# jonassibbesen/rpvg

Measured on AMD Instinct MI355X. Metric: read-pairs quantified/sec, higher is better.
Workload: dtype f64

## Files before the change

### rpvg_amd/csrc/bounded_search.hip

```cpp

#include "common.hpp"
#include "search_plan.hpp"

#include <algorithm>
#include <cstdlib>
#include <map>
#include <memory>
#include <mutex>
#include <numeric>

using namespace rpvg_hip_detail;
using namespace rpvg_search;

namespace {
std::mutex g_search_gate_mutex;
const rpvg_hip_ctx * g_search_gate_owner = nullptr;
}

static bool searchLaunchesEarly() {
    static const bool early = RPVG_EXPERIMENT_ENV("RPVG_HIP_SEARCH_LAUNCH_EARLY") != nullptr;
    return early;
}

constexpr uint64_t kSearchGateRows = 1ull << 17;

static void searchGateEnter(rpvg_hip_ctx * ctx, hipStream_t stream, const uint64_t matrix_rows) {
    static const bool open_gate = RPVG_EXPERIMENT_ENV("RPVG_HIP_NO_SEARCH_GATE") != nullptr;
    ctx->search_gate_held = !open_gate && matrix_rows >= kSearchGateRows;
    if (!ctx->search_gate_held) return;
    hipEvent_t previous = nullptr;
    {
        std::lock_guard<std::mutex> lock(g_search_gate_mutex);
        if (g_search_gate_owner && g_search_gate_owner != ctx && g_search_gate_owner->device == ctx->device) {
            previous = g_search_gate_owner->search_done;
            (void) hipStreamWaitEvent(stream, previous, 0);
        }
    }
    if (previous && !searchLaunchesEarly()) (void) waitEvent(previous);
}

static void searchGateLeave(rpvg_hip_ctx * ctx, hipStream_t stream) {
    if (!ctx->search_gate_held) return;
    ctx->search_gate_held = false;
    std::lock_guard<std::mutex> lock(g_search_gate_mutex);
    (void) hipEventRecord(ctx->search_done, stream);
    g_search_gate_owner = ctx;
}

void searchGateForget(const rpvg_hip_ctx * ctx) {
    std::lock_guard<std::mutex> lock(g_search_gate_mutex);
    if (g_search_gate_owner == ctx) g_search_gate_owner = nullptr;
}

struct rpvg_hip_pair_posteriors {
    std::vector<uint64_t> pair_off;
    void * block = nullptr;
    bool block_pinned = false;
    const uint32_t * first = nullptr, * second = nullptr;
    const double * posterior = nullptr;
    ~rpvg_hip_pair_posteriors() {
        if (block && block_pinned) pinnedFree(block);
        else std::free(block);
    }
};

namespace {

constexpr uint32_t kLdsRows = 2048;
constexpr uint32_t kSmallRowLdsCols = 128;
constexpr uint32_t kRowLdsCols = 512;

__device__ __forceinline__ double waveSum(double v) { return waveSumF64(v); }

__device__ __forceinline__ double addLog(const double log_x, const double log_y) {
    return log_x > log_y ? log_x + log1p(exp(log_y - log_x)) : log_y + log1p(exp(log_x - log_y));
}


template <int kBlock, typename ValueFn>
__device__ __forceinline__ double blockLogSumExp(const uint32_t n, ValueFn value, double * scratch) {
    const double lowest = -1.7976931348623157e308;
    const int lane = threadIdx.x & 63, wave = threadIdx.x >> 6;
    double mx = lowest;
    for (uint32_t k = threadIdx.x; k < n; k += kBlock) mx = fmax(mx, value(k));
#pragma unroll
    for (int d = 32; d >= 1; d >>= 1) mx = fmax(mx, __shfl_xor(mx, d, 64));
    __syncthreads();
    if (lane == 0) scratch[wave] = mx;
    __syncthreads();
#pragma unroll
    for (int w2 = 0; w2 < kBlock / 64; ++w2) mx = fmax(mx, scratch[w2]);
    double sum = 0.0;
    for (uint32_t k = threadIdx.x; k < n; k += kBlock) {
        const double v = value(k);
        if (v > lowest) sum += exp(v - mx);
    }
    sum = waveSum(sum);
    __syncthreads();
    if (lane == 0) scratch[wave] = sum;
    __syncthreads();
    double total = 0.0;
#pragma unroll
    for (int w2 = 0; w2 < kBlock / 64; ++w2) total += scratch[w2];
    return (n == 0 || !(mx > lowest)) ? lowest : mx + log(total);
}

struct SearchArgs {
    const uint32_t * order;
    uint32_t count;
    GroupMatricesView g;
    const uint64_t * col_off;
    const uint32_t * col_count;
    const uint64_t * pair_cap_off;
    double min_log_likelihood_diff;
    uint32_t stage_rows;
    uint32_t row_lds_cols;
    double * log_freq;
    double * marginal;
    double * optimistic_raw;
    double * optimistic;
    uint32_t * col_order;
    uint32_t * out_first;
    uint32_t * out_second;
    double * out_value;
    uint32_t * out_count;
    unsigned long long * log_evals;
};

constexpr int kTileFirst = 4;

template <int kGroup>
__device__ __forceinline__ void tilePairSums(const LogTableEntry * lt, const double * lds_count, const double * lds_base, const uint32_t stride,
                                             const double * __restrict__ cnt, const double * __restrict__ nz,
                                             const double * const (&col_a)[kTileFirst], const double * __restrict__ col_b, const uint32_t staged,
// ... 769 lines not shown
        pair_off[m] = run;
        run += counts[m];
    }
    if (threadIdx.x == 1023) pair_off[num_matrices] = sums[1023];
    if (threadIdx.x == 0 && build_error) *build_error_out = *build_error;
    __syncthreads();
    for (uint32_t i = threadIdx.x; i < tail_words; i += blockDim.x) tail_copy[i] = counts[i];
}

__global__ void compactPairsBlockKernel(const uint32_t num_matrices, const uint64_t * __restrict__ pair_cap_off,
                                        const uint64_t * __restrict__ pair_off, const uint32_t * __restrict__ in_first,
                                        const uint32_t * __restrict__ in_second, const double * __restrict__ in_value,
                                        unsigned char * __restrict__ block) {
    const uint32_t m = blockIdx.x;
    if (m >= num_matrices) return;
    const uint64_t total = pair_off[num_matrices];
    double * out_value = reinterpret_cast<double *>(block);
    uint32_t * out_first = reinterpret_cast<uint32_t *>(block + total * sizeof(double));
    uint32_t * out_second = out_first + total;
    const uint64_t src = pair_cap_off[m], dst = pair_off[m], n = pair_off[m + 1] - pair_off[m];
    for (uint64_t k = threadIdx.x; k < n; k += blockDim.x) {
        out_first[dst + k] = in_first[src + k];
        out_second[dst + k] = in_second[src + k];
        out_value[dst + k] = in_value[src + k];
    }
}


PairSearchKnobs pairSearchKnobs() {
    PairSearchKnobs knobs;
    if (const char * env = std::getenv("RPVG_HIP_PAIR_TILES")) knobs.tiles_wanted = std::atoi(env);
    if (const char * env = std::getenv("RPVG_HIP_TABLE_MIN_WORK")) knobs.table_min_work = std::atof(env);
    if (const char * env = std::getenv("RPVG_HIP_PAIR_CHUNK_ROWS")) knobs.chunk_rows = std::max(256, std::atoi(env));
    return knobs;
}

int searchFailed(const hipError_t e) {
    setError("rpvg_hip_bounded_pair_posteriors: %s", hipGetErrorString(e));
    return (e == hipErrorOutOfMemory) ? RPVG_HIP_ERR_ALLOC : RPVG_HIP_ERR_RUNTIME;
}

void showSearchClasses(const rpvg_hip_groups * groups, const PairSearchPlan & plan) {
    const std::vector<uint32_t> & order = plan.order;
    const uint32_t M = static_cast<uint32_t>(order.size()), num_big = plan.num_big, num_medium = plan.num_medium;
    auto show = [&](const char * name, uint32_t first, uint32_t count) {
        double evals = 0;
        for (uint32_t i = first; i < first + count; ++i) evals += 0.5 * groups->h_num_rows[order[i]] * groups->h_num_cols[order[i]] * groups->h_num_cols[order[i]];
        std::fprintf(stderr, "[search classes] %-6s %6u matrices, %.3g pair-row evaluations if nothing is skipped; largest:", name, count, evals);
        for (uint32_t i = first; i < first + std::min<uint32_t>(count, 6); ++i) std::fprintf(stderr, " %llux%u", static_cast<unsigned long long>(groups->h_num_rows[order[i]]), groups->h_num_cols[order[i]]);
        std::fprintf(stderr, "\n");
    };
    show("table", 0, num_big);
    if (plan.pair_tiles) {
        struct Bucket { uint64_t matrices = 0; double rows = 0, evals = 0, lane_rows = 0, slot_rows = 0; };
        std::map<uint32_t, Bucket> buckets;
        for (uint32_t i = 0; i < num_big; ++i) {
            const double R = static_cast<double>(groups->h_num_rows[order[i]]);
            const uint32_t G = groups->h_num_cols[order[i]];
            uint32_t key = 1;
            while (key < G) key <<= 1;
            Bucket & b = buckets[key];
            const uint32_t tiles = tileCount(G);
            b.matrices += 1;
            b.rows += R;
            b.evals += R * (0.5 * G * (G + 1));
            std::vector<std::pair<uint32_t, uint32_t> > ranges;
            planTileRanges(tiles, &ranges);
            for (auto & range : ranges) b.lane_rows += R / (kTileBlock / range.second) * kTileBlock;
            b.slot_rows += R * tiles * 16;
        }
        for (auto & kv : buckets) {
            const Bucket & b = kv.second;
            std::fprintf(stderr, "[search classes]   columns <= %4u: %6llu matrices, %9.0f rows, %.3g evaluations, pairs / tile slots %.2f, tile slots / lane slots %.2f\n",
                         kv.first, static_cast<unsigned long long>(b.matrices), b.rows, b.evals, b.evals / b.slot_rows, b.slot_rows / (16.0 * b.lane_rows));
        }
    }
    show("medium", num_big, num_medium);
    show("small", num_big + num_medium, M - num_big - num_medium);
}

unsigned long long * searchLogEvals(const PairSearchWork & w) { return reinterpret_cast<unsigned long long *>(w.d_tail.ptr + w.evals_word); }

hipError_t launchTablePart(rpvg_hip_ctx * ctx, const rpvg_hip_groups * groups, const GroupMatricesView & view, const PairSearchPlan & plan,
                           PairSearchWork & w, const bool runs_behind_search) {
    hipError_t e = hipSuccess;
    auto ok = [&](hipError_t r) { if (e == hipSuccess) e = r; return e == hipSuccess; };
    hipStream_t st = ctx->stream;
    const SearchParts parts = {w.d_part_pair.ptr, w.d_part_marg.ptr, w.d_part_opt.ptr, w.d_big_pair_part_off.ptr, w.d_big_col_part_off.ptr, plan.chunk_rows};
    const uint32_t items = static_cast<uint32_t>(plan.item_matrix.size());
    if (plan.pair_tiles) {
        PairTileWork pw;
        pw.item_matrix = w.d_item_matrix.ptr;
        pw.item_chunk = w.d_item_chunk.ptr;
        pw.item_tiles = w.d_item_col.ptr;
        pw.count = items;
        pw.g = view;
        pw.parts = parts;
        pw.log_evals = searchLogEvals(w);
#ifdef RPVG_HIP_EXPERIMENTS
        pw.debug_skip = RPVG_EXPERIMENT_ENV("RPVG_HIP_PAIR_DEBUG") ? static_cast<uint32_t>(std::atoi(RPVG_EXPERIMENT_ENV("RPVG_HIP_PAIR_DEBUG"))) : 0u;
#endif
        static const size_t tile_lds_bytes = []() {
            const char * env = RPVG_EXPERIMENT_ENV("RPVG_HIP_PAIR_LDS_KB");
            return std::max<size_t>(kTileLdsDoubles * sizeof(double), env ? static_cast<size_t>(std::atoi(env)) * 1024 : 0);
        }();
        if (tile_lds_bytes > 64 * 1024) {
            e = hipFuncSetAttribute(reinterpret_cast<const void *>(&pairTile2Kernel), hipFuncAttributeMaxDynamicSharedMemorySize, static_cast<int>(tile_lds_bytes));
            if (e != hipSuccess) return e;
        }
        const int tile_span = ctx->spanBegin(FAM_TILE, st);
        pairTile2Kernel<<<dim3(pw.count), dim3(kTileBlock), tile_lds_bytes, st>>>(pw);
        ctx->spanEnd(tile_span);
#ifdef RPVG_HIP_EXPERIMENTS
        for (int k = RPVG_EXPERIMENT_ENV("RPVG_HIP_PAIR_REPEAT") ? std::atoi(RPVG_EXPERIMENT_ENV("RPVG_HIP_PAIR_REPEAT")) : 0; k > 0; --k) {
            pairTile2Kernel<<<dim3(pw.count), dim3(kTileBlock), tile_lds_bytes, st>>>(pw);
        }
#endif
    } else {
        TableWork tw;
        tw.item_matrix = w.d_item_matrix.ptr;
        tw.item_col = w.d_item_col.ptr;
        tw.item_chunk = w.d_item_chunk.ptr;
        tw.count = items;
        tw.g = view;
        tw.parts = parts;
        tw.log_evals = searchLogEvals(w);
        pairTableKernel<<<dim3(((tw.count + 7) / 8) * 8), dim3(256), 0, st>>>(tw);
    }
    if (runs_behind_search) {
        if (groups->collapse_done) {
            HostScope wait_scope("search: wait for the runs of the matrices' collapse");
            ok(searchLaunchesEarly() ? hipStreamWaitEvent(st, groups->collapse_done, 0) : waitEvent(groups->collapse_done));
        }
        ok(groups->held_back_runs(st, &parts));
        groups->held_back_runs = nullptr;
    }

    ResolveArgs ra;
    ra.big_matrix = w.d_order.ptr;
    ra.count = plan.num_big;
    ra.g = view;
    ra.col_off = w.d_col_off.ptr;
    ra.col_count = w.d_col_count.ptr;
    ra.pair_cap_off = w.d_pair_cap_off.ptr;
    ra.parts = parts;
    ra.min_log_likelihood_diff = w.min_log_likelihood_diff;
    ra.log_freq = w.d_lf.ptr;
    ra.marginal = w.d_marg.ptr;
    ra.col_order = w.d_col_order.ptr;
    ra.seq_value = w.d_seq.ptr;
    ra.out_first = w.d_out_first.ptr;
    ra.out_second = w.d_out_second.ptr;
    ra.out_value = w.d_out_value.ptr;
    ra.out_count = w.d_tail.ptr;
    resolveTableKernel<<<dim3(plan.num_big), dim3(256), 0, st>>>(ra);
    return e;
}

void launchSequentialParts(rpvg_hip_ctx * ctx, const GroupMatricesView & view, const PairSearchPlan & plan, PairSearchWork & w) {
    static const int search_streams = []() {
        const char * env = RPVG_EXPERIMENT_ENV("RPVG_HIP_SEARCH_STREAMS");
        return env ? std::max(1, std::min(3, std::atoi(env))) : 3;
    }();
    hipStream_t s_medium = search_streams == 1 ? ctx->stream : ctx->aux[0];
    hipStream_t s_small = search_streams == 1 ? ctx->stream : (search_streams == 2 ? ctx->aux[0] : ctx->aux[1]);
    SearchArgs args;
    args.g = view;
    args.col_off = w.d_col_off.ptr;
    args.col_count = w.d_col_count.ptr;
    args.pair_cap_off = w.d_pair_cap_off.ptr;
    args.min_log_likelihood_diff = w.min_log_likelihood_diff;
    args.log_freq = w.d_lf.ptr;
    args.marginal = w.d_marg.ptr;
    args.optimistic_raw = w.d_opt_raw.ptr;
    args.optimistic = w.d_opt.ptr;
    args.col_order = w.d_col_order.ptr;
    args.out_first = w.d_out_first.ptr;
    args.out_second = w.d_out_second.ptr;
    args.out_value = w.d_out_value.ptr;
    args.out_count = w.d_tail.ptr;
    args.log_evals = searchLogEvals(w);
    auto search_lds_bytes = [](uint32_t stage_rows, uint32_t row_cols) { return static_cast<size_t>((kTileFirst + 1) * stage_rows + kTileFirst * row_cols) * sizeof(double); };
    {
        static std::once_flag once;
        std::call_once(once, [&]() {
            (void) hipFuncSetAttribute(reinterpret_cast<const void *>(&boundedSearchKernel<1024, 64>), hipFuncAttributeMaxDynamicSharedMemorySize,
                                       static_cast<int>(search_lds_bytes(kLdsRows, kRowLdsCols)));
        });
    }
    const uint32_t num_small = w.M - plan.num_big - plan.num_medium;
    if (plan.num_medium > 0) {
        args.order = w.d_order.ptr + plan.num_big;
        args.count = plan.num_medium;
        args.stage_rows = kLdsRows;
        args.row_lds_cols = kRowLdsCols;
        boundedSearchKernel<1024, 64><<<dim3(plan.num_medium), dim3(1024), search_lds_bytes(kLdsRows, kRowLdsCols), s_medium>>>(args);
    }
    if (num_small > 0) {
        args.order = w.d_order.ptr + plan.num_big + plan.num_medium;
        args.count = num_small;
        args.stage_rows = kSmallRows;
        args.row_lds_cols = kSmallRowLdsCols;
        boundedSearchKernel<256, 16><<<dim3(num_small), dim3(256), search_lds_bytes(kSmallRows, kSmallRowLdsCols), s_small>>>(args);
    }
}

}

namespace rpvg_hip_detail {

int queuePairSearch(rpvg_hip_ctx * ctx, const rpvg_hip_groups * groups, const uint32_t * column_counts, const double min_rel_likelihood,
                    PairSearchWork & w) {
    std::unique_ptr<HostScope> scope(new HostScope("bounded search: host order + work items"));
    const uint32_t M = groups->num_matrices;
    w.M = M;
    w.min_log_likelihood_diff = std::log(min_rel_likelihood);
    if (!column_counts && M > 0 && !groups->d_column_counts) {
        setError("rpvg_hip_bounded_pair_posteriors: column_counts is NULL");
        return RPVG_HIP_ERR_INVALID;
    }
    const uint64_t num_columns = std::accumulate(groups->h_num_cols.begin(), groups->h_num_cols.begin() + M, uint64_t(0));
    for (uint64_t c = 0; column_counts && c < num_columns; ++c) {
        if (column_counts[c] == 0) {
            setError("rpvg_hip_bounded_pair_posteriors: column %llu has a zero count", static_cast<unsigned long long>(c));
            return RPVG_HIP_ERR_INVALID;
        }
    }
    w.plan = planPairSearch(groups->h_num_rows.data(), groups->h_num_cols.data(), M, min_rel_likelihood, pairSearchKnobs());
    const PairSearchPlan & plan = w.plan;
    if (RPVG_EXPERIMENT_ENV("RPVG_HIP_SEARCH_CLASSES")) showSearchClasses(groups, plan);

    scope.reset(new HostScope("bounded search: uploads + launches"));
    hipError_t e = hipSetDevice(ctx->device);
    hipStream_t st = ctx->stream;
    auto ok = [&](hipError_t r) { if (e == hipSuccess) e = r; return e == hipSuccess; };

    UploadPack & pack = w.pack;
    const uint64_t columns = plan.col_off[M], pair_cap = plan.pair_cap_off[M];
    pack.add(w.d_order, plan.order.data(), M);
    pack.add(w.d_col_off, plan.col_off.data(), M + 1);
    pack.add(w.d_pair_cap_off, plan.pair_cap_off.data(), M + 1);
    if (column_counts) pack.add(w.d_col_count, column_counts, columns);
    if (plan.num_big > 0) {
        pack.add(w.d_item_matrix, plan.item_matrix.data(), plan.item_matrix.size());
        pack.add(w.d_item_col, plan.item_col.data(), plan.item_col.size());
        pack.add(w.d_item_chunk, plan.item_chunk.data(), plan.item_chunk.size());
        pack.add(w.d_big_col_part_off, plan.big_col_part_off.data(), M);
        pack.add(w.d_big_pair_part_off, plan.big_pair_part_off.data(), M);
    }
    w.evals_word = (M + 1) & ~1u;
    w.tail_words = w.evals_word + 4;
    pack.addZero(w.d_tail, w.tail_words);
    if (w.extra_u64_count) pack.add(w.d_extra_u64, w.extra_u64, w.extra_u64_count);
    if (w.extra_zero_bytes) pack.addZero(w.d_extra_zero, w.extra_zero_bytes);
    int span = ctx->spanBegin(FAM_H2D);
    ok(pack.commit(st));
    if (!column_counts) w.d_col_count.borrow(const_cast<uint32_t *>(groups->d_column_counts), columns);
    ctx->spanEnd(span);
    ctx->stats.h2d_bytes += static_cast<double>(M * 20 + columns * 4);
    ok(w.d_lf.alloc(columns));
    ok(w.d_marg.alloc(columns));
    ok(w.d_opt_raw.alloc(columns));
    ok(w.d_opt.alloc(columns));
    ok(w.d_col_order.alloc(columns));
    ok(w.d_out_first.alloc(pair_cap));
    ok(w.d_out_second.alloc(pair_cap));
    ok(w.d_out_value.alloc(pair_cap));
    if (e != hipSuccess) return searchFailed(e);
    if (plan.num_big > 0) {
        ok(w.d_part_marg.alloc(plan.col_part_total));
        ok(w.d_part_opt.alloc(plan.col_part_total));
        ok(w.d_part_pair.alloc(plan.pair_part_total));
        ok(w.d_seq.alloc(pair_cap));
    }
    if (e != hipSuccess) return searchFailed(e);

    const bool side_kernels = M > plan.num_big;
    const bool runs_behind_search = static_cast<bool>(groups->held_back_runs) && plan.pair_tiles && plan.num_big == M;
    if (!runs_behind_search) {
        ok(groups->waitCollapse(st));
        if (groups->collapse_done && !searchLaunchesEarly()) {
            HostScope wait_scope("search: wait for the collapse of the matrices");
            ok(waitEvent(groups->collapse_done));
        }
    }
    span = ctx->spanBegin(FAM_LOGLIK);
    searchGateEnter(ctx, st, std::accumulate(groups->h_num_rows.begin(), groups->h_num_rows.end(), uint64_t(0)));
    if (side_kernels) ok(ctx->forkAux());
    const GroupMatricesView view = groups->view();
    if (plan.num_big > 0) ok(launchTablePart(ctx, groups, view, plan, w, runs_behind_search && e == hipSuccess));
    launchSequentialParts(ctx, view, plan, w);
    if (side_kernels) ok(ctx->joinAux());
    ctx->spanEnd(span);
    ctx->stats.loglik_launches += (plan.num_big > 0 ? 2 : 0) + (plan.num_medium > 0) + (M > plan.num_big + plan.num_medium);
    ok(hipGetLastError());
    if (e != hipSuccess) {
        (void) hipStreamSynchronize(st);
        searchFailed(e);
        return RPVG_HIP_ERR_RUNTIME;
    }
    return RPVG_HIP_OK;
}

void leavePairSearch(rpvg_hip_ctx * ctx) { searchGateLeave(ctx, ctx->stream); }

void accountPairSearch(rpvg_hip_ctx * ctx, const rpvg_hip_groups * groups, const PairSearchWork & w, const unsigned long long log_evals,
                       const uint64_t kept_pairs) {
    ctx->stats.loglik_evals += static_cast<double>(log_evals);
    for (uint32_t i = 0; i < w.M; ++i) {
        const double G = groups->h_num_cols[w.plan.order[i]];
        ctx->stats.search_pairs_possible += G * (G + 1) / 2;
        if (i < w.plan.num_big) ctx->stats.search_pairs_table += G * (G + 1) / 2;
    }
    ctx->stats.search_pairs_kept += static_cast<double>(kept_pairs);
}

}

extern "C" int rpvg_hip_bounded_pair_posteriors(rpvg_hip_ctx * ctx, const rpvg_hip_groups * groups,
                                                const uint32_t * column_counts, double min_rel_likelihood,
                                                rpvg_hip_pair_posteriors ** result_out) {
    RPVG_REQUIRE(ctx && groups && result_out, "rpvg_hip_bounded_pair_posteriors: NULL argument");
    *result_out = nullptr;
    RPVG_REQUIRE(min_rel_likelihood > 0, "rpvg_hip_bounded_pair_posteriors: min_rel_likelihood must be positive");
    const uint32_t M = groups->num_matrices;
    rpvg_hip_pair_posteriors * res = new (std::nothrow) rpvg_hip_pair_posteriors();
    if (!res) {
        setError("rpvg_hip_bounded_pair_posteriors: out of host memory");
        return RPVG_HIP_ERR_ALLOC;
    }
    res->pair_off.assign(M + 1, 0);
    if (M == 0) {
        *result_out = res;
        return RPVG_HIP_OK;
    }
    if (!column_counts && !groups->d_column_counts) {
        delete res;
        setError("rpvg_hip_bounded_pair_posteriors: column_counts is NULL");
        return RPVG_HIP_ERR_INVALID;
    }

    std::lock_guard<std::mutex> lock(ctx->mutex);
    PairSearchWork w;
    {
        const int rc = queuePairSearch(ctx, groups, column_counts, min_rel_likelihood, w);
        if (rc != RPVG_HIP_OK) {
            delete res;
            return rc;
        }
    }
    hipError_t e = hipSuccess;
    hipStream_t st = ctx->stream;
    auto ok = [&](hipError_t r) { if (e == hipSuccess) e = r; return e == hipSuccess; };
    std::unique_ptr<HostScope> scope;
    const std::vector<uint64_t> & pair_cap_off = w.plan.pair_cap_off;
    const uint32_t evals_word = w.evals_word, tail_words = w.tail_words;
    auto & d_tail = w.d_tail; auto & d_pair_cap_off = w.d_pair_cap_off; auto & d_out_first = w.d_out_first;
    auto & d_out_second = w.d_out_second; auto & d_out_value = w.d_out_value;
    DeviceBuffer<uint64_t> d_pair_off;

    const char * with_counts_env = std::getenv("RPVG_HIP_PAIRS_WITH_COUNTS");
    const size_t kPairsWithTheCounts = with_counts_env ? static_cast<size_t>(std::atof(with_counts_env)) : (size_t(1) << 20);
    const size_t tail_bytes = tail_words * sizeof(uint32_t), tail_room = (tail_bytes + 255) & ~size_t(255);
    const size_t block_capacity = static_cast<size_t>(pair_cap_off[M]) * 16;
    const size_t first_copy = tail_room + std::min(block_capacity, kPairsWithTheCounts);
    DeviceBuffer<unsigned char> d_result;
    ok(d_pair_off.alloc(M + 1));
    ok(d_result.alloc(tail_room + block_capacity));
    void * host_result = nullptr;
    if (e == hipSuccess && pinnedAlloc(&host_result, first_copy) != hipSuccess) e = hipErrorOutOfMemory;
    if (e == hipSuccess) {
        const bool check_build = !groups->build_checked && groups->build_error_flag.ptr;
        pairOffsetsKernel<<<dim3(1), dim3(1024), 0, st>>>(M, d_tail.ptr, d_pair_off.ptr, check_build ? groups->build_error_flag.ptr : nullptr,
                                                         d_tail.ptr + evals_word + 2, reinterpret_cast<uint32_t *>(d_result.ptr), tail_words);
        compactPairsBlockKernel<<<dim3(M), dim3(64), 0, st>>>(M, d_pair_cap_off.ptr, d_pair_off.ptr, d_out_first.ptr, d_out_second.ptr,
                                                             d_out_value.ptr, d_result.ptr + tail_room);
        ok(hipGetLastError());
        ok(hipMemcpyAsync(host_result, d_result.ptr, first_copy, hipMemcpyDeviceToHost, st));
    }
    searchGateLeave(ctx, st);
    scope.reset(new HostScope("bounded search: wait for the kernels"));
    ok(waitStream(st));
    if (e == hipSuccess) {
        const uint32_t * counts = static_cast<const uint32_t *>(host_result);
        unsigned long long log_evals = 0;
        std::memcpy(&log_evals, counts + evals_word, sizeof(log_evals));
        const uint32_t build_bad = counts[evals_word + 2];
        for (uint32_t m = 0; m < M; ++m) res->pair_off[m + 1] = res->pair_off[m] + counts[m];
        if (build_bad) {
            pinnedFree(host_result);
            delete res;
            setError(build_bad == 2 ? "rpvg_hip_groups_build: a group lists a path twice" : "rpvg_hip_groups_build: a group refers to a path outside its cluster");
            return RPVG_HIP_ERR_INVALID;
        }
        groups->build_checked = true;
        const uint64_t total = res->pair_off[M];
        const unsigned char * pairs = nullptr;
        if (total * 16 <= first_copy - tail_room) {
            res->block = host_result;
            res->block_pinned = true;
            host_result = nullptr;
            pairs = static_cast<const unsigned char *>(res->block) + tail_room;
        } else {
            scope.reset(new HostScope("bounded search: download pairs"));
            if (pinnedAlloc(&res->block, total * 16) == hipSuccess) {
                res->block_pinned = true;
            } else {
                res->block = std::malloc(total * 16);
                if (!res->block) e = hipErrorOutOfMemory;
            }
            if (e == hipSuccess) {
                ok(hipMemcpyAsync(res->block, d_result.ptr + tail_room, total * 16, hipMemcpyDeviceToHost, st));
                ok(waitStream(st));
                pairs = static_cast<const unsigned char *>(res->block);
            }
        }
        if (e == hipSuccess) {
            res->posterior = reinterpret_cast<const double *>(pairs);
            res->first = reinterpret_cast<const uint32_t *>(pairs + total * sizeof(double));
            res->second = res->first + total;
        }
        accountPairSearch(ctx, groups, w, log_evals, total);
    }
    if (host_result) pinnedFree(host_result);
    if (e != hipSuccess) {
        delete res;
        return searchFailed(e);
    }
    *result_out = res;
    return RPVG_HIP_OK;
}

extern "C" int rpvg_hip_pair_posteriors_get(const rpvg_hip_pair_posteriors * result, rpvg_hip_pair_posteriors_view * view_out) {
    RPVG_REQUIRE(result && view_out, "rpvg_hip_pair_posteriors_get: NULL argument");
    view_out->num_matrices = static_cast<uint32_t>(result->pair_off.size() - 1);
    view_out->pair_off = result->pair_off.data();
    view_out->first = result->first;
    view_out->second = result->second;
    view_out->posterior = result->posterior;
    return RPVG_HIP_OK;
}

extern "C" void rpvg_hip_pair_posteriors_free(rpvg_hip_pair_posteriors * result) { delete result; }
```

### rpvg_amd/csrc/common.hpp

```cpp
#ifndef RPVG_HIP_COMMON_HPP
#define RPVG_HIP_COMMON_HPP

#include <hip/hip_runtime.h>

#include <algorithm>
#include <chrono>
#include <cstdarg>
#include <cstdint>
#include <cstdio>
#include <cstdlib>
#include <cstring>
#include <memory>
#include <mutex>
#include <new>
#include <string>
#include <functional>
#include <vector>

#include "../../include/rpvg_hip.h"
#include "search_plan.hpp"
#include "em_plan.hpp"
#include "batch_forms.hpp"

namespace rpvg_hip_detail {
// ... 417 lines not shown
        for (int t = 0; t < kOut; ++t) acc[t] = fma(c, logPositive(xs[t], lt), acc[t]);
    }
}

constexpr int kCollapseKeyFractionBits = 22;
constexpr int kCollapseProjectionBits = kCollapseKeyFractionBits + 2;
constexpr int kCollapseLargestBits = 20;
constexpr int kCollapseLargestFractionBits = 27;
constexpr int kCollapseMatrixShift = kCollapseProjectionBits + kCollapseLargestBits;
constexpr uint32_t kCollapseMaxMatrices = 1u << 20;

__host__ __device__ inline double collapseWeight(const uint32_t column) {
    return static_cast<double>(((column * 0x9E3779B1u) >> 8) & 0xFFFFu) * (1.0 / 32768.0);
}

__host__ __device__ inline uint64_t collapseSortKey(const uint32_t matrix, const double key, const double largest) {
    const double k = key < 0.0 ? 0.0 : (key > 3.999999 ? 3.999999 : key);
    const double l = largest < 0.0 ? 0.0 : (largest > 0.999999 ? 0.999999 : largest);
    return (static_cast<uint64_t>(matrix) << kCollapseMatrixShift) |
           (static_cast<uint64_t>(k * static_cast<double>(1ull << kCollapseKeyFractionBits)) << kCollapseLargestBits) |
           (static_cast<uint64_t>(l * static_cast<double>(1ull << kCollapseLargestFractionBits)) & ((1ull << kCollapseLargestBits) - 1));
}

__device__ __forceinline__ double mulRounded(const double a, const double b) {
#pragma clang fp contract(off)
    return a * b;
}
__device__ __forceinline__ double addRounded(const double a, const double b) {
#pragma clang fp contract(off)
    return a + b;
}

template <int BLOCK>
__device__ __forceinline__ uint32_t blockExclusiveSum(const uint32_t v, uint32_t & total, uint32_t * scratch) {
    const int lane = threadIdx.x & 63, wave = threadIdx.x >> 6;
    uint32_t incl = v;
#pragma unroll
    for (int d = 1; d < 64; d <<= 1) {
        const uint32_t up = __shfl_up(incl, d, 64);
        if (lane >= d) incl += up;
    }
    __syncthreads();
    if (lane == 63) scratch[wave] = incl;
    __syncthreads();
    uint32_t before = 0, all = 0;
#pragma unroll
    for (int w = 0; w < BLOCK / 64; ++w) {
        if (w < wave) before += scratch[w];
        all += scratch[w];
    }
    total = all;
    return before + incl - v;
}

enum KernelFamily { FAM_EM_SPARSE = 0, FAM_EM_DENSE, FAM_LOGLIK, FAM_BUILD, FAM_H2D, FAM_COLLAPSE, FAM_EM_KERNEL, FAM_GIBBS, FAM_TILE, FAM_COUNT };

struct TimedSpan {
    hipEvent_t start, stop;
    int family;
    int sub;
};

struct TimedInterval {
    double start_ms, stop_ms;
    int family;
    uint64_t clock;
};

}

namespace rpvg_hip_detail {
struct SubsetEmHints {
    double subsets_per_matrix = 0, list_per_path = 0, rows_per_row = 0, entries_per_entry = 0;
    bool retry = false;
    unsigned long long retry_subsets = 0, retry_list_length = 0, retry_rows = 0, retry_entries = 0;
};
}

struct rpvg_hip_ctx {
    static constexpr int kAuxStreams = 6;
    rpvg_hip_detail::SubsetEmHints subset_hints;
    rpvg_hip_detail::SubsetEmHints subset_full_hints;
    bool search_gate_held = false;
    int device = 0;
    hipStream_t stream = nullptr;
    hipStream_t aux[kAuxStreams] = {};
    int aux_count = kAuxStreams;
    hipStream_t grid_stream[2] = {nullptr, nullptr};
    hipEvent_t grid_ready = nullptr;
    hipStream_t collapse_stream = nullptr;
    hipStream_t copy_stream = nullptr;
    hipEvent_t copied = nullptr;
    hipEvent_t fork_event = nullptr;
    hipEvent_t search_done = nullptr;
    hipEvent_t join_event[kAuxStreams] = {};
    hipError_t forkAux();
    hipError_t joinAux();
    hipError_t joinAuxOnHost();
    hipDeviceProp_t props;
    std::mutex mutex;
    void * comm = nullptr;
    int comm_world = 1, comm_rank = 0;
    int allReduceSumF64(double * device_buf, uint64_t n);
    std::vector<rpvg_hip_detail::TimedSpan> spans;
    std::vector<hipStream_t> span_streams;
    int span_level = 2;
    int open_spans = 0;
    void accountSpan(const rpvg_hip_detail::TimedSpan & span, const void * clock_base, uint64_t clock_id);
    void foldFinishedSpans();
    std::vector<rpvg_hip_detail::TimedInterval> intervals;
    rpvg_hip_kernel_stats stats;

    int spanBegin(int family, hipStream_t on = nullptr, int sub = -1);
    void spanEnd(int idx);
    int foldSpans();
};

namespace rpvg_hip_detail {
struct PathSourcesPending {
    DeviceBuffer<uint64_t> d_path_source_off;
    DeviceBuffer<uint32_t> d_source_id, d_sizes;
    DeviceBuffer<uint16_t> d_source_id16;
    DeviceBuffer<unsigned long long> d_arena;
    unsigned long long arena_words = 0, num_sources = 0, num_sources_narrow = 0;
    void * h_sizes = nullptr;
    uint32_t K = 0;
    bool copied = false, queued = false;
    ~PathSourcesPending() { if (h_sizes) pinnedFree(h_sizes); }
};
}

struct rpvg_hip_batch {
    uint32_t num_clusters = 0;
    uint64_t num_rows = 0, num_entries = 0, num_paths = 0;
    std::vector<uint64_t> h_cluster_row_off, h_cluster_path_off, h_cluster_ent_off;
    rpvg_hip_detail::DeviceBuffer<uint64_t> cluster_row_off;
    rpvg_hip_detail::DeviceBuffer<uint64_t> cluster_path_off;
    rpvg_hip_detail::DeviceBuffer<double> row_count;
    rpvg_hip_detail::DeviceBuffer<double> row_noise;
    rpvg_hip_detail::DeviceBuffer<uint64_t> row_ent_off;
    rpvg_hip_detail::DeviceBuffer<uint32_t> ent_path;
    rpvg_hip_detail::DeviceBuffer<double> ent_prob;
    std::vector<double> h_cluster_total;
    bool has_source_columns = false;
    rpvg_hip_detail::DeviceBuffer<uint32_t> path_group_id;
    rpvg_hip_detail::DeviceBuffer<uint64_t> cluster_src_off;
    rpvg_hip_detail::DeviceBuffer<uint32_t> src_col_count;
    rpvg_hip_detail::DeviceBuffer<uint32_t> src_col_end;
    rpvg_hip_detail::DeviceBuffer<uint32_t> src_col_path;
    std::vector<uint64_t> h_cluster_src_off;
    std::vector<uint32_t> h_src_num_cols, h_src_col_paths, h_src_max_col_paths;
    struct UploadInProgress {
        rpvg_batch_forms::BatchForms forms;
        rpvg_hip_detail::DeviceBuffer<uint32_t> d_row_count_u32, d_row_grp_off32, d_grp_idx_off32;
        rpvg_hip_detail::DeviceBuffer<uint64_t> d_row_grp_off, d_grp_idx_off;
        rpvg_hip_detail::DeviceBuffer<double> d_grp_prob;
        rpvg_hip_detail::DeviceBuffer<uint8_t> d_row_grp_count8, d_grp_idx_count8;
        rpvg_hip_detail::DeviceBuffer<uint16_t> d_path_idx16, d_row_noise16;
        rpvg_hip_detail::DeviceBuffer<double> d_row_noise_table;
        rpvg_hip_detail::DeviceBuffer<uint8_t> d_row_count8;
        rpvg_hip_detail::DeviceBuffer<uint32_t> d_escape_row, d_escape_count;
        rpvg_hip_detail::PathSourcesPending path_sources;
        rpvg_hip_detail::DeviceBuffer<unsigned long long> d_first_bad_row;
        rpvg_hip_detail::DeviceBuffer<double> d_cluster_total;
        rpvg_hip_detail::DeviceBuffer<uint64_t> d_cluster_ent_off;
        rpvg_hip_detail::DeviceBuffer<unsigned char> scan_scratch_rows, scan_scratch_groups;
// ... 240 lines not shown
    EmProblemsView problems;
    double * abundances;
    double * noise_count;
    uint32_t * iterations;
    const EmFusedDense * fused = nullptr;
    uint32_t num_fused = 0;
};

uint64_t emGridMinWork();
uint64_t gibbsGridMinWork();
bool emGridDenseRoute(uint32_t columns, uint32_t rows, uint32_t entries);
int runEmGridProblems(rpvg_hip_ctx * ctx, hipStream_t st, const EmGridProblem * problems, uint32_t count, const EmGridStorage & storage,
                      uint32_t max_em_its, double max_rel_em_conv);

struct GibbsGridProblem {
    uint32_t problem, columns;
    uint32_t rows, entries;
    uint32_t num_samples, pad;
    uint64_t col_begin;
    uint64_t sample_off, abund_sample_off;
    uint64_t seed;
};
struct GibbsGridStorage {
    EmProblemsView problems;
    const double * init_abundances;
    const double * init_noise_count;
    double * noise_samples;
    double * abundance_samples;
};
int runGibbsGridProblems(rpvg_hip_ctx * ctx, hipStream_t st, const GibbsGridProblem * problems, uint32_t count, const GibbsGridStorage & storage,
                         uint32_t gibbs_thin_its, double gamma);

struct DenseEmRun {
    const double * matrix = nullptr;
    uint64_t num_rows = 0;
    uint32_t num_cols = 0;
    uint64_t ld = 0;
    const double * counts = nullptr;
    double total_count = 0, zero_mass = 0;
    uint32_t max_em_its = 0;
    double max_rel_em_conv = 0;
    bool sharded = false;
    DeviceBuffer<double> d_a;
    EmGridControl control = {};
};
int emDenseIterate(rpvg_hip_ctx * ctx, const char * who, DenseEmRun & run);

int queueEmSolve(rpvg_hip_ctx * ctx, const rpvg_hip_batch * batch, const EmProblemList & list, uint32_t max_em_its,
                 double max_rel_em_conv, const EmOutputs & out, EmSolveWork & work, double collapse_precision = 0.0);
EmSolveKnobs emSolveKnobs();
int queueEmFill(rpvg_hip_ctx * ctx, const rpvg_hip_batch * batch, const EmProblemList & list, const EmOutputs & out, EmSolveWork & work,
                const EmSolveKnobs & knobs, const EmFillPlan & plan, bool fused_look, int & build_span);
EmSolveShape emSolveShape(const rpvg_hip_ctx * ctx, const EmProblemList & list, bool collapse_wanted);

struct HostProblemSet {
    EmProblemList list;
    EmSolveWork work;
    DeviceBuffer<uint32_t> d_cluster, d_col_path, d_item_problem;
    DeviceBuffer<uint64_t> d_col_off, d_row_base, d_ent_base, d_seg_first;
    UploadPack uploads;
    uint64_t n_cols_total = 0;
};
int prepareHostProblems(rpvg_hip_ctx * ctx, const rpvg_hip_batch * batch, const rpvg_hip_em_problems * problems,
                        HostProblemSet & ps, const EmOutputs & out, const char * who);
void accountEmSolve(rpvg_hip_ctx * ctx, uint32_t P, const uint64_t * col_off, const uint32_t * kept_rows, const uint32_t * kept_entries,
                    const uint32_t * iterations);

struct PairSearchWork {
    uint32_t M = 0, evals_word = 0, tail_words = 0;
    double min_log_likelihood_diff = 0;
    rpvg_search::PairSearchPlan plan;
    DeviceBuffer<uint32_t> d_order, d_col_count, d_col_order, d_out_first, d_out_second, d_item_matrix, d_item_col, d_item_chunk;
    DeviceBuffer<uint32_t> d_tail;
    DeviceBuffer<uint64_t> d_col_off, d_pair_cap_off, d_big_col_part_off, d_big_pair_part_off;
    DeviceBuffer<double> d_lf, d_marg, d_opt_raw, d_opt, d_out_value, d_part_marg, d_part_opt, d_part_pair, d_seq;
    UploadPack pack;
    const uint64_t * extra_u64 = nullptr;
    size_t extra_u64_count = 0, extra_zero_bytes = 0;
    DeviceBuffer<uint64_t> d_extra_u64;
    DeviceBuffer<unsigned char> d_extra_zero;
};
int queuePairSearch(rpvg_hip_ctx * ctx, const rpvg_hip_groups * groups, const uint32_t * column_counts, double min_rel_likelihood,
                    PairSearchWork & w);
void leavePairSearch(rpvg_hip_ctx * ctx);
void accountPairSearch(rpvg_hip_ctx * ctx, const rpvg_hip_groups * groups, const PairSearchWork & w, unsigned long long log_evals, uint64_t kept_pairs);

struct CsrCollapseInput {
    uint32_t num_problems_bound = 0;
    const uint32_t * num_problems_dev = nullptr;
    uint64_t rows_capacity = 0;
    EmProblemsView problems;
    uint32_t num_items_bound = 0;
    const uint32_t * num_items_dev = nullptr;
    const uint64_t * seg_first = nullptr;
    const uint32_t * item_problem = nullptr;
    uint32_t segment_rows = 0;
    uint64_t max_rows_bound = 0;
};
struct CsrCollapseWork {
    DeviceBuffer<double> merged_count;
    DeviceBuffer<uint32_t> problem_merged;
    DeviceBuffer<uint32_t> info;
    std::shared_ptr<void> temporaries;
};
hipError_t queueCsrCollapse(rpvg_hip_ctx * ctx, const CsrCollapseInput & in, double precision, CsrCollapseWork & work, hipStream_t stream,
                            hipEvent_t sorted = nullptr);

std::unique_ptr<rpvg_hip_batch> newBatchShell(uint32_t num_clusters, uint64_t num_rows, uint64_t num_entries, uint64_t num_paths, hipError_t & e);
struct GroupedRows {
    uint64_t num_groups = 0;
    const void * row_grp_off = nullptr;
    const void * grp_idx_off = nullptr;
    bool row_off32 = false, grp_off32 = false;
    const double * grp_prob = nullptr;
    const uint32_t * row_count_u32 = nullptr;
};
hipError_t queueGroupedRows(hipStream_t stream, const GroupedRows & rows, rpvg_hip_batch * b, unsigned long long * d_first_bad_row, uint64_t * d_cluster_ent_off);

hipError_t queueClusterTotals(hipStream_t stream, uint32_t num_clusters, const uint64_t * d_cluster_row_off, const uint32_t * d_row_count_u32, double * d_totals);
hipError_t queuePathSourceCopies(rpvg_hip_ctx * ctx, rpvg_hip_batch * b, const rpvg_cluster_batch * hb, PathSourcesPending & pending);
hipError_t queuePathSourceKernels(rpvg_hip_ctx * ctx, rpvg_hip_batch * b, PathSourcesPending & pending, hipStream_t stream);
hipError_t reservePathSources(rpvg_hip_batch * b, uint32_t num_clusters, uint64_t num_paths, uint64_t num_sources, PathSourcesPending & pending);
int finishPathSources(rpvg_hip_batch * b, PathSourcesPending & pending);

hipError_t queueRowCollapse(rpvg_hip_ctx * ctx, rpvg_hip_groups * groups, uint64_t total_rows, double precision, hipStream_t stream, bool hold_back_runs = false);
}

#endif
```

### rpvg_amd/csrc/subset_em.hip

```cpp

#include "common.hpp"
#include "subset_pack.hpp"

#include <cmath>
#include <memory>

using namespace rpvg_hip_detail;

namespace {

constexpr uint32_t kMaxSelected = 1024;

struct MergedList {
    const uint32_t * a;
    const uint32_t * b;
    uint32_t na, nb, i, j;
    __device__ __forceinline__ MergedList(const uint32_t * a_in, uint32_t na_in, const uint32_t * b_in, uint32_t nb_in)
        : a(a_in), b(b_in), na(na_in), nb(nb_in), i(0), j(0) {}
    __device__ __forceinline__ bool done() const { return i >= na && j >= nb; }
    __device__ __forceinline__ uint32_t next() {
        if (j >= nb || (i < na && a[i] <= b[j])) return a[i++];
        return b[j++];
    }
};
// ... 539 lines not shown
        cap_subsets = std::min<unsigned long long>(slots, std::max(cap_subsets, hints.retry_subsets + 64));
        cap_length = std::max(cap_length, hints.retry_list_length + 64);
        cap_rows = std::max(cap_rows, hints.retry_rows + 64);
        cap_entries = std::max(cap_entries, hints.retry_entries + 64);
        hints.retry = false;
    }
    const unsigned long long cap_columns = cap_length;
    const unsigned long long cap_items = cap_rows / emFillSegmentRows() + cap_subsets;

    scope.reset(new HostScope("subset em: search + kernels queued"));
    const size_t header_room = 256;
    int rc = RPVG_HIP_OK;
    if (!second_attempt) {
        search.extra_u64 = slot_off.data();
        search.extra_u64_count = M + 1;
        search.extra_zero_bytes = header_room + emQueuesBytes();
        rc = queuePairSearch(ctx, groups, column_counts, min_rel_likelihood, search);
        if (rc != RPVG_HIP_OK) return rc;
    } else {
        const hipError_t zeroed = zeroAsync(search.d_extra_zero.ptr, search.extra_zero_bytes, st);
        if (zeroed != hipSuccess) {
            setError("rpvg_hip_nested_subset_em: %s", hipGetErrorString(zeroed));
            return RPVG_HIP_ERR_RUNTIME;
        }
    }

    hipError_t e = hipSuccess;
    auto ok = [&](hipError_t r) { if (e == hipSuccess) e = r; return e == hipSuccess; };
    const uint64_t * d_slot_off = search.d_extra_u64.ptr;
    SubsetHeader * header = reinterpret_cast<SubsetHeader *>(search.d_extra_zero.ptr);
    static_assert(sizeof(SubsetHeader) <= 256, "room for the header");
    DeviceBuffer<uint32_t> d_slot_first, d_slot_second, d_slot_length, d_slot_columns;
    DeviceBuffer<double> d_slot_weight;
    DeviceBuffer<unsigned char> d_totals, d_bases, d_packed;
    ok(d_slot_first.alloc(slots));
    ok(d_slot_second.alloc(slots));
    ok(d_slot_length.alloc(slots));
    ok(d_slot_columns.alloc(slots));
    ok(d_slot_weight.alloc(slots));
    ok(d_totals.alloc(sizeof(MatrixTotals) * M));
    ok(d_bases.alloc(sizeof(MatrixTotals) * M));
    DeviceBuffer<uint32_t> d_big_matrices;
    ok(d_big_matrices.alloc(M));
    DeviceBuffer<uint32_t> d_sub_cluster, d_path, d_col_path, d_iters, d_kept_rows, d_kept_entries;
    DeviceBuffer<double> d_sub_weight, d_abund, d_noise, d_total;
    DeviceBuffer<uint64_t> d_path_off, d_col_off, d_row_base, d_ent_base, d_subset_off, d_seg_first;
    DeviceBuffer<uint32_t> d_item_problem;
    ok(d_sub_cluster.alloc(cap_subsets));
    ok(d_sub_weight.alloc(cap_subsets));
    ok(d_path_off.alloc(cap_subsets + 1));
    ok(d_col_off.alloc(cap_subsets + 1));
    ok(d_row_base.alloc(cap_subsets));
    ok(d_ent_base.alloc(cap_subsets));
    ok(d_subset_off.alloc(M + 1));
    ok(d_seg_first.alloc(cap_subsets + 1));
    ok(d_item_problem.alloc(cap_items));
    ok(d_path.alloc(cap_length));
    ok(d_col_path.alloc(cap_columns));
    ok(d_abund.alloc(cap_columns));
    ok(d_noise.alloc(cap_subsets));
    ok(d_total.alloc(cap_subsets));
    ok(d_iters.alloc(cap_subsets));
    ok(d_kept_rows.alloc(cap_subsets));
    ok(d_kept_entries.alloc(cap_subsets));
    const size_t packed_capacity = packedLayout(M, cap_subsets, cap_length, cap_columns).bytes;
    ok(d_packed.alloc(packed_capacity));
    const bool merge_here = batch->path_group_id.ptr != nullptr && max_paths < (1u << kMergePathBits) - 2;
    DeviceBuffer<unsigned long long> d_merge_key;
    DeviceBuffer<uint32_t> d_merge_pos;
    DeviceBuffer<double> d_merge_a0, d_merge_a1;
    if (merge_here) {
        ok(d_merge_key.alloc(2 * cap_length + 2));
        ok(d_merge_pos.alloc(2 * cap_length + 2));
        ok(d_merge_a0.alloc(cap_length));
        ok(d_merge_a1.alloc(cap_length));
    }
    void * pinned_header = nullptr;
    if (e == hipSuccess && pinnedAlloc(&pinned_header, sizeof(SubsetHeader)) != hipSuccess) e = hipErrorOutOfMemory;
    hipEvent_t header_here = nullptr;
    if (e == hipSuccess) ok(hipEventCreateWithFlags(&header_here, hipEventDisableTiming));
    if (e != hipSuccess) {
        setError("rpvg_hip_nested_subset_em: %s", hipGetErrorString(e));
        (void) hipStreamSynchronize(st);
        leavePairSearch(ctx);
        if (pinned_header) pinnedFree(pinned_header);
        if (header_here) (void) hipEventDestroy(header_here);
        return (e == hipErrorOutOfMemory) ? RPVG_HIP_ERR_ALLOC : RPVG_HIP_ERR_RUNTIME;
    }
    MatrixTotals * totals = reinterpret_cast<MatrixTotals *>(d_totals.ptr);
    MatrixTotals * bases = reinterpret_cast<MatrixTotals *>(d_bases.ptr);

    std::unique_ptr<HostScope> part_scope(new HostScope("subset em: select + offsets + expand queued"));
    int span = ctx->spanBegin(FAM_BUILD);
    SelectArgs sa;
    sa.num_matrices = M;
    sa.pair_count = search.d_tail.ptr;
    sa.pair_cap_off = search.d_pair_cap_off.ptr;
    sa.pair_first = search.d_out_first.ptr;
    sa.pair_second = search.d_out_second.ptr;
    sa.pair_value = search.d_out_value.ptr;
    sa.group_off = groups->d_group_off;
    sa.group_path_off = groups->d_group_path_off;
    sa.group_path = groups->d_group_path;
    sa.cluster = groups->d_cluster;
    sa.mat_rows = groups->mat_rows.ptr;
    sa.cluster_row_off = batch->cluster_row_off.ptr;
    sa.row_ent_off = batch->row_ent_off.ptr;
    sa.slot_off = d_slot_off;
    sa.min_hap_prob = min_hap_prob;
    sa.segment_rows = emFillSegmentRows();
    sa.slot_first = d_slot_first.ptr;
    sa.slot_second = d_slot_second.ptr;
    sa.slot_weight = d_slot_weight.ptr;
    sa.slot_length = d_slot_length.ptr;
    sa.slot_columns = d_slot_columns.ptr;
    sa.totals = totals;
    sa.header = header;
    sa.big_matrices = d_big_matrices.ptr;
    subsetSelectSmallKernel<<<dim3(M), dim3(64), 0, st>>>(sa);
    subsetSelectWideKernel<<<dim3(std::min<uint32_t>(M, 128)), dim3(256), 0, st>>>(sa);
    const bool check_build = !groups->build_checked && groups->build_error_flag.ptr;
    OffsetsArgs oa;
    oa.pair_count = search.d_tail.ptr;
    oa.log_evals = reinterpret_cast<const unsigned long long *>(search.d_tail.ptr + search.evals_word);
    oa.build_error = check_build ? groups->build_error_flag.ptr : nullptr;
    oa.num_matrices = M;
    oa.totals = totals;
    oa.bases = bases;
    oa.header = header;
    oa.cap_subsets = cap_subsets;
    oa.cap_length = cap_length;
    oa.cap_columns = cap_columns;
    oa.cap_rows = cap_rows;
    oa.cap_entries = cap_entries;
    oa.cap_items = cap_items;
    oa.seg_first = d_seg_first.ptr;
    oa.path_off = d_path_off.ptr;
    oa.col_off = d_col_off.ptr;
    subsetOffsetsKernel<<<dim3(1), dim3(1024), 0, st>>>(oa);
    SubsetHeader * h_header = static_cast<SubsetHeader *>(pinned_header);
    ok(hipMemcpyAsync(h_header, header, sizeof(SubsetHeader), hipMemcpyDeviceToHost, st));
    ok(hipEventRecord(header_here, st));
    ExpandArgs ea;
    ea.num_matrices = M;
    ea.header = header;
    ea.totals = totals;
    ea.bases = bases;
    ea.slot_off = d_slot_off;
    ea.slot_first = d_slot_first.ptr;
    ea.slot_second = d_slot_second.ptr;
    ea.slot_weight = d_slot_weight.ptr;
    ea.slot_length = d_slot_length.ptr;
    ea.slot_columns = d_slot_columns.ptr;
    ea.group_off = groups->d_group_off;
    ea.group_path_off = groups->d_group_path_off;
    ea.group_path = groups->d_group_path;
    ea.cluster = groups->d_cluster;
    ea.cluster_row_off = batch->cluster_row_off.ptr;
    ea.row_ent_off = batch->row_ent_off.ptr;
    ea.sub_cluster = d_sub_cluster.ptr;
    ea.sub_weight = d_sub_weight.ptr;
    ea.path_off = d_path_off.ptr;
    ea.path = d_path.ptr;
    ea.col_off = d_col_off.ptr;
    ea.col_path = d_col_path.ptr;
    ea.row_base = d_row_base.ptr;
    ea.ent_base = d_ent_base.ptr;
    ea.seg_first = d_seg_first.ptr;
    ea.item_problem = d_item_problem.ptr;
    ea.segment_rows = emFillSegmentRows();
    ea.subset_off = d_subset_off.ptr;
    subsetExpandKernel<<<dim3(M), dim3(256), 0, st>>>(ea);
    ok(hipGetLastError());
    ctx->spanEnd(span);
    ctx->stats.build_launches += 4;
    leavePairSearch(ctx);

    part_scope.reset();
    EmProblemList list;
    list.P_bound = static_cast<uint32_t>(std::min<unsigned long long>(cap_subsets, 0xfffffffeull));
    list.d_num_problems = &header->num_problems;
    list.d_cluster = d_sub_cluster.ptr;
    list.d_col_off = d_col_off.ptr;
    list.d_col_path = d_col_path.ptr;
    list.d_row_base = d_row_base.ptr;
    list.d_ent_base = d_ent_base.ptr;
    list.rows_capacity = cap_rows;
    list.entries_capacity = cap_entries;
    list.d_seg_first = d_seg_first.ptr;
    list.d_item_problem = d_item_problem.ptr;
    list.items_bound = static_cast<uint32_t>(std::min<unsigned long long>(cap_items, 0xfffffffeull));
    list.d_num_items = &header->num_items;
    list.max_cols = max_paths + 1;
    list.max_cluster_paths = max_paths;
    list.max_cluster_work = max_cluster_work;
    list.wide_capacity = 0;
    EmOutputs out{d_abund.ptr, d_noise.ptr, d_iters.ptr, d_kept_rows.ptr, d_kept_entries.ptr, d_total.ptr};
    EmSolveWork work;
    work.zeroed_queues = search.d_extra_zero.ptr + header_room;
    if (e == hipSuccess) {
        rc = queueEmSolve(ctx, batch, list, max_em_its, max_rel_em_conv, out, work, collapse_precision);
        if (rc != RPVG_HIP_OK) {
            (void) hipStreamSynchronize(st);
            (void) hipEventDestroy(header_here);
            pinnedFree(pinned_header);
            return rc;
        }
    }
    part_scope.reset(new HostScope("subset em: merge + pack queued"));
    static_assert(sizeof(SubsetHeader) <= 192, "the merge's flag word sits behind the header");
    uint32_t * d_merge_bad = reinterpret_cast<uint32_t *>(search.d_extra_zero.ptr + 192);
    if (merge_here && e == hipSuccess) {
        MergeArgs ma;
        ma.header = header;
        ma.num_matrices = M;
        ma.subset_off = d_subset_off.ptr;
        ma.weight = d_sub_weight.ptr;
        ma.path_off = d_path_off.ptr;
        ma.path = d_path.ptr;
        ma.col_off = d_col_off.ptr;
        ma.col_path = d_col_path.ptr;
        ma.abundances = d_abund.ptr;
        ma.noise = d_noise.ptr;
        ma.total = d_total.ptr;
        ma.cluster = groups->d_cluster;
        ma.cluster_path_off = batch->cluster_path_off.ptr;
        ma.path_group_id = batch->path_group_id.ptr;
        ma.sort_key = d_merge_key.ptr;
        ma.sort_pos = d_merge_pos.ptr;
        ma.rec_a0 = d_merge_a0.ptr;
        ma.rec_a1 = d_merge_a1.ptr;
        ma.merge_bad = d_merge_bad;
        ma.packed = d_packed.ptr;
        const int merge_span = ctx->spanBegin(FAM_BUILD);
        subsetMergeKernel<<<dim3(M), dim3(256), 0, st>>>(ma);
        ctx->spanEnd(merge_span);
        ctx->stats.build_launches += 1;
    }
    PackArgs pa;
    pa.merge_bad = merge_here ? d_merge_bad : nullptr;
    pa.header = header;
    pa.num_matrices = M;
    pa.subset_off = d_subset_off.ptr;
    pa.weight = d_sub_weight.ptr;
    pa.path_off = d_path_off.ptr;
    pa.col_off = d_col_off.ptr;
    pa.abundances = d_abund.ptr;
    pa.noise = d_noise.ptr;
    pa.total = d_total.ptr;
    pa.path = d_path.ptr;
    pa.col_path = d_col_path.ptr;
    pa.iterations = d_iters.ptr;
    pa.kept_rows = d_kept_rows.ptr;
    pa.kept_entries = d_kept_entries.ptr;
    pa.packed = d_packed.ptr;
    packResultsKernel<<<dim3(256), dim3(256), 0, st>>>(pa);
    ok(hipGetLastError());

    part_scope.reset();
// ... 117 lines not shown
```

Measured before the change: 2.458 billion.

## Turn search gate into ticketed per-device chain and publish right after tile kernels

The cross-context search gate becomes a per-device FIFO ticket chain: each context takes a ticket, waits on a condition variable until its predecessor has published, and orders its stream behind that predecessor's done event. The gate is now released as soon as the search kernels are queued (right after the tile kernel when there are no side kernels) instead of after the subset EM build or the bounded search copy. The aim is to let the next context's large search start earlier and overlap with this context's later stages. In exchange it adds host-side blocking on the condition variable, and a context that takes a ticket and never publishes would stall the others.

Result: no change. 2.470 billion, median of 2 (+0.5%).

```diff
diff --git a/rpvg_amd/csrc/bounded_search.hip b/rpvg_amd/csrc/bounded_search.hip
--- a/rpvg_amd/csrc/bounded_search.hip
+++ b/rpvg_amd/csrc/bounded_search.hip
@@ -3,6 +3,7 @@
 #include "search_plan.hpp"
 
 #include <algorithm>
+#include <condition_variable>
 #include <cstdlib>
 #include <map>
 #include <memory>
@@ -13,8 +14,13 @@
 using namespace rpvg_search;
 
 namespace {
+struct SearchGateChain {
+    uint64_t entered = 0, published = 0;
+    const rpvg_hip_ctx * last = nullptr;
+};
 std::mutex g_search_gate_mutex;
-const rpvg_hip_ctx * g_search_gate_owner = nullptr;
+std::condition_variable g_search_gate_published;
+std::map<int, SearchGateChain> g_search_gate_chains;
 }
 
 static bool searchLaunchesEarly() {
@@ -30,26 +36,35 @@
     if (!ctx->search_gate_held) return;
     hipEvent_t previous = nullptr;
     {
-        std::lock_guard<std::mutex> lock(g_search_gate_mutex);
-        if (g_search_gate_owner && g_search_gate_owner != ctx && g_search_gate_owner->device == ctx->device) {
-            previous = g_search_gate_owner->search_done;
+        std::unique_lock<std::mutex> lock(g_search_gate_mutex);
+        SearchGateChain & chain = g_search_gate_chains[ctx->device];
+        ctx->search_gate_ticket = ++chain.entered;
+        g_search_gate_published.wait(lock, [&]() { return chain.published + 1 == ctx->search_gate_ticket; });
+        if (chain.last && chain.last != ctx) {
+            previous = chain.last->search_done;
             (void) hipStreamWaitEvent(stream, previous, 0);
         }
     }
     if (previous && !searchLaunchesEarly()) (void) waitEvent(previous);
 }
 
-static void searchGateLeave(rpvg_hip_ctx * ctx, hipStream_t stream) {
+static void searchGatePublish(rpvg_hip_ctx * ctx, hipStream_t stream) {
     if (!ctx->search_gate_held) return;
     ctx->search_gate_held = false;
-    std::lock_guard<std::mutex> lock(g_search_gate_mutex);
-    (void) hipEventRecord(ctx->search_done, stream);
-    g_search_gate_owner = ctx;
+    {
+        std::lock_guard<std::mutex> lock(g_search_gate_mutex);
+        SearchGateChain & chain = g_search_gate_chains[ctx->device];
+        (void) hipEventRecord(ctx->search_done, stream);
+        chain.published = ctx->search_gate_ticket;
+        chain.last = ctx;
+    }
+    g_search_gate_published.notify_all();
 }
 
 void searchGateForget(const rpvg_hip_ctx * ctx) {
     std::lock_guard<std::mutex> lock(g_search_gate_mutex);
-    if (g_search_gate_owner == ctx) g_search_gate_owner = nullptr;
+    auto chain = g_search_gate_chains.find(ctx->device);
+    if (chain != g_search_gate_chains.end() && chain->second.last == ctx) chain->second.last = nullptr;
 }
 
 struct rpvg_hip_pair_posteriors {
@@ -985,7 +1000,7 @@
 unsigned long long * searchLogEvals(const PairSearchWork & w) { return reinterpret_cast<unsigned long long *>(w.d_tail.ptr + w.evals_word); }
 
 hipError_t launchTablePart(rpvg_hip_ctx * ctx, const rpvg_hip_groups * groups, const GroupMatricesView & view, const PairSearchPlan & plan,
-                           PairSearchWork & w, const bool runs_behind_search) {
+                           PairSearchWork & w, const bool runs_behind_search, const bool publish_behind_tiles) {
     hipError_t e = hipSuccess;
     auto ok = [&](hipError_t r) { if (e == hipSuccess) e = r; return e == hipSuccess; };
     hipStream_t st = ctx->stream;
@@ -1030,6 +1045,7 @@
         tw.log_evals = searchLogEvals(w);
         pairTableKernel<<<dim3(((tw.count + 7) / 8) * 8), dim3(256), 0, st>>>(tw);
     }
+    if (publish_behind_tiles) searchGatePublish(ctx, st);
     if (runs_behind_search) {
         if (groups->collapse_done) {
             HostScope wait_scope("search: wait for the runs of the matrices' collapse");
@@ -1191,9 +1207,10 @@
     searchGateEnter(ctx, st, std::accumulate(groups->h_num_rows.begin(), groups->h_num_rows.end(), uint64_t(0)));
     if (side_kernels) ok(ctx->forkAux());
     const GroupMatricesView view = groups->view();
-    if (plan.num_big > 0) ok(launchTablePart(ctx, groups, view, plan, w, runs_behind_search && e == hipSuccess));
+    if (plan.num_big > 0) ok(launchTablePart(ctx, groups, view, plan, w, runs_behind_search && e == hipSuccess, !side_kernels));
     launchSequentialParts(ctx, view, plan, w);
     if (side_kernels) ok(ctx->joinAux());
+    searchGatePublish(ctx, st);
     ctx->spanEnd(span);
     ctx->stats.loglik_launches += (plan.num_big > 0 ? 2 : 0) + (plan.num_medium > 0) + (M > plan.num_big + plan.num_medium);
     ok(hipGetLastError());
@@ -1204,8 +1221,6 @@
     }
     return RPVG_HIP_OK;
 }
-
-void leavePairSearch(rpvg_hip_ctx * ctx) { searchGateLeave(ctx, ctx->stream); }
 
 void accountPairSearch(rpvg_hip_ctx * ctx, const rpvg_hip_groups * groups, const PairSearchWork & w, const unsigned long long log_evals,
                        const uint64_t kept_pairs) {
@@ -1281,7 +1296,6 @@
         ok(hipGetLastError());
         ok(hipMemcpyAsync(host_result, d_result.ptr, first_copy, hipMemcpyDeviceToHost, st));
     }
-    searchGateLeave(ctx, st);
     scope.reset(new HostScope("bounded search: wait for the kernels"));
     ok(waitStream(st));
     if (e == hipSuccess) {
diff --git a/rpvg_amd/csrc/common.hpp b/rpvg_amd/csrc/common.hpp
--- a/rpvg_amd/csrc/common.hpp
+++ b/rpvg_amd/csrc/common.hpp
@@ -523,6 +523,7 @@
     rpvg_hip_detail::SubsetEmHints subset_hints;
     rpvg_hip_detail::SubsetEmHints subset_full_hints;
     bool search_gate_held = false;
+    uint64_t search_gate_ticket = 0;
     int device = 0;
     hipStream_t stream = nullptr;
     hipStream_t aux[kAuxStreams] = {};
@@ -929,7 +930,6 @@
 };
 int queuePairSearch(rpvg_hip_ctx * ctx, const rpvg_hip_groups * groups, const uint32_t * column_counts, double min_rel_likelihood,
                     PairSearchWork & w);
-void leavePairSearch(rpvg_hip_ctx * ctx);
 void accountPairSearch(rpvg_hip_ctx * ctx, const rpvg_hip_groups * groups, const PairSearchWork & w, unsigned long long log_evals, uint64_t kept_pairs);
 
 struct CsrCollapseInput {
diff --git a/rpvg_amd/csrc/subset_em.hip b/rpvg_amd/csrc/subset_em.hip
--- a/rpvg_amd/csrc/subset_em.hip
+++ b/rpvg_amd/csrc/subset_em.hip
@@ -645,7 +645,6 @@
     if (e != hipSuccess) {
         setError("rpvg_hip_nested_subset_em: %s", hipGetErrorString(e));
         (void) hipStreamSynchronize(st);
-        leavePairSearch(ctx);
         if (pinned_header) pinnedFree(pinned_header);
         if (header_here) (void) hipEventDestroy(header_here);
         return (e == hipErrorOutOfMemory) ? RPVG_HIP_ERR_ALLOC : RPVG_HIP_ERR_RUNTIME;
@@ -737,7 +736,6 @@
     ok(hipGetLastError());
     ctx->spanEnd(span);
     ctx->stats.build_launches += 4;
-    leavePairSearch(ctx);
 
     part_scope.reset();
     EmProblemList list;
```
